# PeihaoChen/WS-MGMap

Hardware: AMD Instinct MI355X
Metric: policy steps/sec (fwd+bwd), CMA batch=8 seq=64 (higher is better)
Workload: dtype bf16

## Files before the change

include/wsmgmap.h:

```cpp
#ifndef WSMGMAP_H
#define WSMGMAP_H

#include <stdint.h>

#ifdef __cplusplus
extern "C" {
#endif

typedef void* wsmg_stream_t;

#define WSMG_EINVAL (-1)
#define WSMG_ENOMEM (-2)

int wsmg_abi_version(void);
const char* wsmg_build_info(void);


int wsmg_bev_index(const float* depth, int B, int Hd, int Wd, float depth_scale, int Hf, int Wf, int E,
                   float local_scale, int32_t* lin_idx, wsmg_stream_t stream);

int wsmg_bev_scatter_max(const float* feat, const int32_t* lin_idx, int B, int Cf, int Hf, int Wf, int C,
                         int E, float* out, wsmg_stream_t stream);

int wsmg_bev_rotate(const float* in, const float* heading, float sign, int B, int C, int E, float* out,
// ... 258 lines not shown
int wsmg_weight_relayout_bf16(const float* w_oihw, int O, int I, int KH, int KW, int I_pad, void* w_ohwi, void* w_ihwo,
                              wsmg_stream_t stream);
int wsmg_weight_grad_to_oihw(const float* dw_ohwi, int O, int I, int KH, int KW, int I_pad, float* dw_oihw,
                             wsmg_stream_t stream);

int wsmg_conv2d_bwd_weight_bf16_plan(int B, int H, int W, int Cin, int Cout, int KH, int KW, int stride, int pad, int OH, int OW,
                                     int* nsplit, long long* ws_floats);
int wsmg_conv2d_bwd_weight_bf16_slabs(const void* x, const void* dy, float* ws, int nsplit, long long ws_floats, int B, int H, int W,
                                      int Cin, int Cout, int KH, int KW, int stride, int pad, int OH, int OW, wsmg_stream_t stream);
int wsmg_conv2d_bwd_weight_plan(int B, int H, int W, int Cin, int Cout, int KH, int KW, int stride, int pad, int OH, int OW,
                                int* nsplit, long long* ws_floats);
int wsmg_conv2d_bwd_weight_slabs(const float* x, const float* dy, float* ws, int nsplit, long long ws_floats, int B, int H, int W,
                                 int Cin, int Cout, int KH, int KW, int stride, int pad, int OH, int OW, wsmg_stream_t stream);
int wsmg_weight_grad_reduce_oihw(const float* ws, int nsplit, int O, int I, int KH, int KW, int I_pad, float* dw_oihw,
                                 wsmg_stream_t stream);

int wsmg_bn_act_bwd_ld(const float* dy, int64_t ld_dy, const float* x, const float* y, const float* gamma, const float* beta,
                       const float* save_mean, const float* save_invstd, int relu, int64_t rows, int C, float* dx, float* dresidual,
                       float* dgamma, float* dbeta, double* workspace, int64_t workspace_bytes, wsmg_stream_t stream);
int wsmg_bn_act_bwd_ld_bf16(const void* dy, int64_t ld_dy, const void* x, const void* y, const float* gamma, const float* beta,
                            const float* save_mean, const float* save_invstd, int relu, int64_t rows, int C, void* dx,
                            void* dresidual, float* dgamma, float* dbeta, double* workspace, int64_t workspace_bytes,
                            wsmg_stream_t stream);
int wsmg_bn_act_bwd_ld_bf16_lo(const void* dy, int64_t ld_dy, const void* x, const void* y, const float* gamma, const float* beta,
                               const float* save_mean, const float* save_invstd, int relu, int64_t rows, int C, void* dx, void* dx_lo,
                               void* dresidual, float* dgamma, float* dbeta, double* workspace, int64_t workspace_bytes,
                               wsmg_stream_t stream);
int wsmg_relu_bwd_rows_bf16(const void* dy, int64_t ld_dy, const void* y, void* dx, int64_t rows, int C, wsmg_stream_t stream);
int wsmg_upsample2x_bwd_ld(const float* dy, int64_t ld_dy, float* dx, int B, int H, int W, int C, wsmg_stream_t stream);
int wsmg_upsample2x_bwd_ld_bf16(const void* dy, int64_t ld_dy, void* dx, int B, int H, int W, int C, wsmg_stream_t stream);
// ... 205 lines not shown
```

ws-mgmap_amd/csrc/wsmg_layout.hip:

```cpp
#include <type_traits>

#include "wsmg_common.h"

namespace {

template <bool TO_NHWC, class TI, class TO>
__global__ __launch_bounds__(256) void transpose_kernel(const TI* x, TO* y, int C_src, int HW, int C_dst) {
  __shared__ float tile[32][33];
  const int b = blockIdx.z;
  const int tx = threadIdx.x & 31, ty = threadIdx.x >> 5;
  if (TO_NHWC) {
    const int p0 = blockIdx.x * 32, c0 = blockIdx.y * 32;
#pragma unroll
    for (int j = 0; j < 4; ++j) {
      int c = c0 + ty + 8 * j, p = p0 + tx;
      tile[ty + 8 * j][tx] = (c < C_src && p < HW) ? ldf(x + ((size_t)b * C_src + c) * HW + p) : 0.f;
    }
    __syncthreads();
#pragma unroll
    for (int j = 0; j < 4; ++j) {
      int p = p0 + ty + 8 * j, c = c0 + tx;
      if (p < HW && c < C_dst) stf(y + ((size_t)b * HW + p) * C_dst + c, tile[tx][ty + 8 * j]);
    }
  } else {
// ... 75 lines not shown
  weight_relayout_body<T>(d.w_oihw, d.O, d.I, d.KH, d.KW, d.I_pad, (T*)d.w_ohwi, (T*)d.w_ihwo);
}
__global__ __launch_bounds__(256) void weight_grad_to_oihw_kernel(const float* __restrict__ dw, int O, int I, int KH, int KW,
                                                                  int I_pad, float* __restrict__ out) {
  const int64_t n = (int64_t)O * I * KH * KW;
  for (int64_t idx = (int64_t)blockIdx.x * 256 + threadIdx.x; idx < n; idx += (int64_t)gridDim.x * 256) {
    const int kw = (int)(idx % KW);
    int64_t r = idx / KW;
    const int kh = (int)(r % KH); r /= KH;
    const int i = (int)(r % I);
    const int o = (int)(r / I);
    out[idx] = dw[(((int64_t)o * KH + kh) * KW + kw) * I_pad + i];
  }
}

__global__ __launch_bounds__(256) void weight_grad_reduce_oihw_kernel(const float* __restrict__ ws, int nsplit, int64_t slab4, int I,
                                                                      int KH, int KW, int I_pad, float* __restrict__ out) {
  __shared__ f32x4 part[3][64];
  const int ql = threadIdx.x & 63, zp = threadIdx.x >> 6;
  const int64_t q = (int64_t)blockIdx.x * 64 + ql;
  const int per = (nsplit + 3) >> 2;
  const int z0 = zp * per, z1 = z0 + per < nsplit ? z0 + per : nsplit;
  f32x4 acc = {0.f, 0.f, 0.f, 0.f};
  if (q < slab4) {
    const f32x4* p = reinterpret_cast<const f32x4*>(ws) + (int64_t)z0 * slab4 + q;
    int z = z0;
    for (; z + 4 <= z1; z += 4, p += 4 * slab4) {
      const f32x4 a = p[0], b = p[slab4], c = p[2 * slab4], d = p[3 * slab4];
      acc += a; acc += b; acc += c; acc += d;
    }
    for (; z < z1; ++z, p += slab4) acc += p[0];
  }
  if (zp) part[zp - 1][ql] = acc;
  __syncthreads();
  if (zp || q >= slab4) return;
  acc += part[0][ql]; acc += part[1][ql]; acc += part[2][ql];
  const OhwiPos p = ohwi_decode(q * 4, KH, KW, I_pad);
#pragma unroll
  for (int j = 0; j < 4; ++j)
    if (p.i + j < I) out[(((int64_t)p.o * I + p.i + j) * KH + p.kh) * KW + p.kw] = acc[j];
}

template <bool TO_NHWC, class TI, class TO>
int transpose_t(const TI* x, TO* y, int B, int C_src, int H, int W, int C_dst, wsmg_stream_t stream) {
  if (B <= 0 || C_src <= 0 || C_dst <= 0 || H <= 0 || W <= 0 || B > 65535) return WSMG_EINVAL;
  int HW = H * W;
  if constexpr (TO_NHWC && std::is_same<TI, float>::value) {
    if (C_src == C_dst && C_src % 64 == 0 && HW % 4 == 0) {
      dim3 g64((unsigned)wsmg_cdiv(HW, 64), (unsigned)(C_src / 64), (unsigned)B);
      hipLaunchKernelGGL((nchw_to_nhwc64_kernel<TO>), g64, dim3(256), 0, wsmg_s(stream), x, y, C_src, HW, C_dst);
      WSMG_RETURN_LAUNCH();
    }
  }
  dim3 grid((unsigned)wsmg_cdiv(HW, 32), (unsigned)wsmg_cdiv(TO_NHWC ? C_dst : (C_dst > C_src ? C_dst : C_src), 32), (unsigned)B);
  hipLaunchKernelGGL((transpose_kernel<TO_NHWC, TI, TO>), grid, dim3(256), 0, wsmg_s(stream), x, y, C_src, HW, C_dst);
  WSMG_RETURN_LAUNCH();
}

bool weight_shape_ok(int O, int I, int KH, int KW, int I_pad) { return O > 0 && I > 0 && KH > 0 && KW > 0 && I_pad >= I; }

template <class T>
int weight_relayout_t(const float* w_oihw, int O, int I, int KH, int KW, int I_pad, T* w_ohwi, T* w_ihwo, wsmg_stream_t s) {
  if (!weight_shape_ok(O, I, KH, KW, I_pad)) return WSMG_EINVAL;
  hipLaunchKernelGGL(weight_relayout_kernel<T>, dim3(wsmg_sgrid((int64_t)O * KH * KW * I_pad)), dim3(256), 0, wsmg_s(s), w_oihw, O, I, KH,
                     KW, I_pad, w_ohwi, w_ihwo);
  WSMG_RETURN_LAUNCH();
}

}

#define B16(p) ((bf16_t*)(p))
#define CB16(p) ((const bf16_t*)(p))
extern "C" int wsmg_nchw_to_nhwc(const float* x, float* y, int B, int C_src, int H, int W, int C_dst, wsmg_stream_t s) { return transpose_t<true, float, float>(x, y, B, C_src, H, W, C_dst, s); }
extern "C" int wsmg_nchw_to_nhwc_bf16(const float* x, void* y, int B, int C_src, int H, int W, int C_dst, wsmg_stream_t s) { return transpose_t<true, float, bf16_t>(x, B16(y), B, C_src, H, W, C_dst, s); }
extern "C" int wsmg_nhwc_to_nchw(const float* x, float* y, int B, int C_src, int H, int W, int C_dst, wsmg_stream_t s) { return transpose_t<false, float, float>(x, y, B, C_src, H, W, C_dst, s); }
extern "C" int wsmg_nhwc_to_nchw_bf16(const void* x, float* y, int B, int C_src, int H, int W, int C_dst, wsmg_stream_t s) { return transpose_t<false, bf16_t, float>(CB16(x), y, B, C_src, H, W, C_dst, s); }

extern "C" int wsmg_weight_relayout(const float* w_oihw, int O, int I, int KH, int KW, int I_pad, float* w_ohwi, float* w_ihwo, wsmg_stream_t s) { return weight_relayout_t<float>(w_oihw, O, I, KH, KW, I_pad, w_ohwi, w_ihwo, s); }
extern "C" int wsmg_weight_relayout_bf16(const float* w_oihw, int O, int I, int KH, int KW, int I_pad, void* w_ohwi, void* w_ihwo, wsmg_stream_t s) { return weight_relayout_t<bf16_t>(w_oihw, O, I, KH, KW, I_pad, B16(w_ohwi), B16(w_ihwo), s); }
extern "C" int wsmg_weight_relayout_multi(const WsmgRelayoutDesc* descs, int n, int bf16, wsmg_stream_t s) {
  if (!descs || n <= 0) return WSMG_EINVAL;
// ... 5 lines not shown
      if (!weight_shape_ok(d.O, d.I, d.KH, d.KW, d.I_pad) || !d.w_oihw || !d.w_ohwi) return WSMG_EINVAL;
    }
    if (bf16) hipLaunchKernelGGL(weight_relayout_multi_kernel<bf16_t>, dim3(48, (unsigned)m), dim3(256), 0, wsmg_s(s), b);
    else hipLaunchKernelGGL(weight_relayout_multi_kernel<float>, dim3(48, (unsigned)m), dim3(256), 0, wsmg_s(s), b);
  }
  WSMG_RETURN_LAUNCH();
}
extern "C" int wsmg_weight_grad_reduce_oihw(const float* ws, int nsplit, int O, int I, int KH, int KW, int I_pad, float* dw_oihw,
                                            wsmg_stream_t s) {
  if (!ws || !dw_oihw || nsplit <= 0 || !weight_shape_ok(O, I, KH, KW, I_pad) || (I_pad & 3)) return WSMG_EINVAL;
  const int64_t slab4 = (int64_t)O * KH * KW * I_pad / 4;
  hipLaunchKernelGGL(weight_grad_reduce_oihw_kernel, dim3((unsigned)wsmg_cdiv(slab4, 64)), dim3(256), 0, wsmg_s(s), ws, nsplit, slab4, I,
                     KH, KW, I_pad, dw_oihw);
  WSMG_RETURN_LAUNCH();
}
extern "C" int wsmg_weight_grad_to_oihw(const float* dw_ohwi, int O, int I, int KH, int KW, int I_pad, float* dw_oihw, wsmg_stream_t s) {
  if (!weight_shape_ok(O, I, KH, KW, I_pad)) return WSMG_EINVAL;
  hipLaunchKernelGGL(weight_grad_to_oihw_kernel, dim3(wsmg_sgrid((int64_t)O * I * KH * KW)), dim3(256), 0, wsmg_s(s), dw_ohwi, O, I, KH, KW,
                     I_pad, dw_oihw);
  WSMG_RETURN_LAUNCH();
}
```

ws-mgmap_amd/wsmgmap/_abi.py:

```python
import ctypes
import os
import re

_HERE = os.path.dirname(os.path.abspath(__file__))
LIB_PATH = os.path.join(_HERE, "lib", "libwsmgmap.so")
if os.environ.get("WSMG_LIB"):
    LIB_PATH = os.environ["WSMG_LIB"]
HEADER_PATH = os.path.join(os.path.dirname(os.path.dirname(_HERE)), "include", "wsmgmap.h")


class WsmgError(RuntimeError):
    pass


_VALUE_TYPES = {"int": ctypes.c_int, "int32_t": ctypes.c_int, "unsigned": ctypes.c_uint, "uint32_t": ctypes.c_uint,
                "float": ctypes.c_float, "double": ctypes.c_double, "int64_t": ctypes.c_int64, "long long": ctypes.c_longlong,
                "wsmg_stream_t": ctypes.c_void_p}
_RETURN_TYPES = {"int": ctypes.c_int, "int64_t": ctypes.c_int64, "long long": ctypes.c_longlong, "const char*": ctypes.c_char_p}


def _ctype(decl, where):
    if "*" in decl:
        return ctypes.c_void_p
    ty = " ".join(decl.split()[:-1])
# ... 105 lines not shown

def take_rnn_status():
    global rnn_timeouts
    v = int(lib().wsmg_rnn_status(1))
    if v:
        rnn_timeouts += 1
    return v


def status_names(bits):
    return [n for b, n in STATUS_BITS if bits & b]


def exported_names():
    return list(_SIG)
```

ws-mgmap_amd/wsmgmap/debug.py:

```python
import os

_TABLE = [
    ("recurrent_chunks", "WSMG_RECURRENT_CHUNKS", 4, int, "time chunks of the pipelined recurrent core (wsmgmap/recurrent.py); 0 = the staged route"),
    ("rows_gemm", "WSMG_ROWS_GEMM", True, bool, "the recurrent core's dense layers as one launch each (csrc/wsmg_rows_gemm.hip); 0: the GEMM library"),
    ("fp8_fused", "WSMG_FP8_FUSED", True, bool, "ops.attention_fp8_shared as one launch (wsmg_attn_fp8_mfma_fused) where its grid barrier is safe"),
    ("fp8_row_fused", "WSMG_FP8_ROW_FUSED", True, bool, "single-query fp8 attention (one token set per row) as one launch: fold + attention per row (round 6)"),
    ("recurrent_chain", "WSMG_RECURRENT_CHAIN", True, bool, "each recurrence of the pipelined core as ONE launch chained to the attention stage by device-side counters"),
    ("decoder_streams", "WSMG_DECODER_STREAMS", 1, int, "0: map decoder on one stream; 1: side stream unless ranks share a GPU; 2: always"),
    ("early_dedup", "WSMG_EARLY_DEDUP", True, bool, "instruction dedup on its own stream when the producer marked the tokens ready (ops.mark_inputs_ready)"),
    ("early_dedup_dp", "WSMG_EARLY_DEDUP_DP", False, bool, "the early dedup also under a process group (needs the exchange on a policy stream: GradAllReducer(exchange_stream=...))"),
    ("rollout_fold", "WSMG_ROLLOUT_FOLD", True, bool, "rollout map stack with BatchNorm-folded cached operands"),
    ("depth_engine", "WSMG_DEPTH_ENGINE", False, bool, "frozen depth ResNet50 on the bf16 NHWC engine (5 % error: opt-in)"),
    ("fused_cls_tail", "WSMG_FUSED_CLS_TAIL", True, bool, "classifier tail (BN + ReLU + 1x1 + CE + pool) in one pass per direction"),
    ("bn_fused_stats", "WSMG_BN_FUSED_STATS", True, bool, "BatchNorm sums in the producing convolution's epilogue"),
    ("relu_producer_mask", "WSMG_RELU_PRODUCER_MASK", True, bool, "fused-ReLU masks of map_encoded / map_classified_linear in map_cated_linear's backward-data epilogue (round 6)"),
    ("conv_into_cat", "WSMG_CONV_INTO_CAT", True, bool, "map_encoded / map_classified_linear write straight into their slices of the concatenation (round 6)"),
    ("strided_grads", "WSMG_STRIDED_GRADS", True, bool, "channel slices of a concatenation's gradient read in place"),
    ("wgrad_atomics", "WSMG_WGRAD_ATOMICS", False, bool, "weight gradients through float atomics instead of slabs + ordered reduce (not bit-reproducible)"),
    ("conv_splitk", "WSMG_CONV_SPLITK", True, bool, "split-K for rollout-size layers"),
    ("rows_linear", "WSMG_ROWS_LINEAR", True, bool, "one-launch dense layers for <= 16 rows"),
    ("bev_fused", "WSMG_BEV_FUSED", True, bool, "scatter + rotation in one launch, plane-consuming fuse"),
    ("bev_compact", "WSMG_BEV_COMPACT", True, bool, "BEV: the index launch packs the valid sources and the scatter walks only those (round 6)"),
    ("bev_one_launch", "WSMG_BEV_ONE_LAUNCH", -1, int, "BEV: index + scatter + rotation as one launch (wsmg_bev_project) and fuse + retrieve as one (wsmg_map_fuse_retrieve); -1: where profiles/bev_fuse_retrieve.txt has them measured and not slower (fuse + retrieve at B = 1 of E = 100, C = 64, G = 240), 0: never, 1: wherever the shapes allow"),
    ("rnn_stock", "WSMG_RNN_STOCK", False, bool, "the three recurrences on the stock (MIOpen) GRU / LSTM: no persistent kernel at all (bench.py's last fallback; needs recurrent_chunks = 0)"),
    ("rnn_poison", "WSMG_RNN_POISON", False, bool, "NaN-fill the persistent kernels' workspaces first (stress tool)"),
    ("feeder_pin", "WSMG_FEEDER_PIN", True, bool, "register the feeder's shared-memory ring as pinned memory"),
    ("keep_blas", "WSMG_KEEP_BLAS", False, bool, "leave torch's BLAS backend choice alone (default: rocBLAS)"),
]


class Switches:
    def __init__(self):
        self.reload()
# ... 20 lines not shown
```

ws-mgmap_amd/wsmgmap/graph.py:

```python
import torch

from . import _abi, ops
from .common.aux_losses import AuxLosses


def _eager_dedup(owner, enc, tokens, first_call, reuse=False):
    if owner._dd_stream is None:
        owner._dd_stream = torch.cuda.Stream()
    cur = torch.cuda.current_stream()
    if first_call:
        owner._dd_stream.wait_stream(cur)
    with torch.cuda.stream(owner._dd_stream):
        dd = enc.dedup(tokens, reuse=reuse)
    cur.wait_stream(owner._dd_stream)
    for t in dd:
        if t.is_cuda:
            t.record_stream(cur)
    return dd


class GraphedAct:

    def __init__(self, policy, eager_calls=2):
        self.policy = policy
# ... 183 lines not shown
        self._bump_versions()
        rnn_hidden_states.copy_(g["h_out"])
        return g["loss"]

    def _capture(self, observations, rnn_hidden_states, prev_actions, masks, weights, dd):
        obs_s = {k: self._adopt(v) for k, v in observations.items() if torch.is_tensor(v)}
        prev_actions, masks, weights = self._adopt(prev_actions), self._adopt(masks), self._adopt(weights)
        dd_s = (dd[0].clone(), dd[1].clone(), dd[2].clone(), dd[3].clone())
        h_in = rnn_hidden_states.clone()
        obs_c = dict(obs_s)
        obs_c["instruction_dedup"] = dd_s
        torch.cuda.synchronize()
        graph = torch.cuda.CUDAGraph()
        with torch.cuda.graph(graph):
            loss, h_out = self._update(obs_c, h_in, prev_actions, masks, weights)
        if hasattr(self.optimizer, "note_replayed_steps"):
            self.optimizer.note_replayed_steps(-1)
        ops.check_rnn_status()
        return dict(graph=graph, obs=obs_s, dd=dd_s, h_in=h_in, prev=prev_actions, masks=masks, weights=weights, loss=loss, h_out=h_out)
```

ws-mgmap_amd/wsmgmap/ops/conv.py:

```python
import ctypes

import torch

from .. import _abi
from ..debug import sw
from .core import _p, _raw_stream, _stream, _req, _f32, _sfx, _workspace, _rows_of, _conv_out, _launch, _zeros_f32, _prelaid, _join_side_at_end, TokenGradSink
from .nhwc import cat_channels
from .norm import channel_sum



def prelayout_conv_weights(weights, dtype):
    descs, keep = [], []
    for w in weights:
        if w.dim() != 4 or not w.is_cuda or w.dtype != torch.float32 or not w.is_contiguous():
            continue
        O, I, KH, KW = w.shape
        cin_pad = (I + 31) // 32 * 32
        key = (w.data_ptr(), w._version, cin_pad, dtype)
        if key in _prelaid:
            continue
        ohwi = torch.empty(O, KH, KW, cin_pad, device=w.device, dtype=dtype)
        ihwo = torch.empty(cin_pad, KH, KW, O, device=w.device, dtype=dtype)
        _prelaid[key] = (ohwi, ihwo)
# ... 25 lines not shown

_wgrad_ws = {}


def _wgrad_workspace(device, floats):
    key = (device.index, _raw_stream())
    ws = _wgrad_ws.get(key)
    if ws is None or ws.numel() < floats:
        if ws is not None:
            ws.record_stream(torch.cuda.current_stream())
        ws = torch.empty(max(int(floats), 1 << 24), device=device, dtype=torch.float32)
        _wgrad_ws[key] = ws
    return ws


def _weight_grad(sfx, x, dy, dims, fl, Cin_w):
    B, H, W, Cin, Cout, KH, KW, stride, pad, OH, OW = dims
    if sw.wgrad_atomics:
        dw_ohwi = _zeros_f32((Cout, KH, KW, Cin), x.device)
        _launch("wsmg_conv2d_bwd_weight" + sfx, fl, _p(x), _p(dy), _p(dw_ohwi), *dims, _stream())
        return _weight_grad_oihw(dw_ohwi, Cin_w)
    nsplit, floats = ctypes.c_int(0), ctypes.c_longlong(0)
    _abi.call("wsmg_conv2d_bwd_weight" + sfx + "_plan", *dims, ctypes.cast(ctypes.byref(nsplit), ctypes.c_void_p),
              ctypes.cast(ctypes.byref(floats), ctypes.c_void_p))
    ws = _wgrad_workspace(x.device, floats.value)
    _launch("wsmg_conv2d_bwd_weight" + sfx + "_slabs", fl, _p(x), _p(dy), _p(ws), nsplit.value, floats.value, *dims, _stream())
    out = torch.empty(Cout, Cin_w, KH, KW, device=x.device, dtype=torch.float32)
    _launch("wsmg_weight_grad_reduce_oihw", 0.0, _p(ws), nsplit.value, Cout, Cin_w, KH, KW, Cin, _p(out), _stream(),
            prof_as="wsmg_conv2d_bwd_weight" + sfx + "_slabs")
    return out


class ReluSink:

    def __init__(self):
        self.relu = False
        self.masked = False


def _mask_of(mask_z, mask_sinks):
    if mask_z is None or not mask_sinks or not sw.relu_producer_mask or not all(m.relu for m in mask_sinks):
        return None
    for m in mask_sinks:
# ... 21 lines not shown
            _launch("wsmg_conv2d_fwd_bf16_ex", fl, _p(x), _p(w), _p(bias), ctypes.c_void_p(base.data_ptr() + c_off * 2), 2 if relu else 0,
                    None, 0, base.shape[-1], *dims, _stream())
        else:
            y = torch.empty(B, OH, OW, Cout, device=x.device, dtype=x.dtype)
            if sfx and stats is not None:
                _launch("wsmg_conv2d_fwd_bf16_stats", fl, _p(x), _p(w), _p(bias), _p(y), 2 if relu else 0, _p(stats), stats.shape[0],
                        *dims, _stream())
            elif sfx:
                _launch("wsmg_conv2d_fwd_bf16", fl, _p(x), _p(w), _p(bias), _p(y), 2 if relu else 0, *dims, _stream())
            else:
                _launch("wsmg_conv2d_fwd", fl, _p(x), _p(w), _p(bias), _p(y), *dims, _stream())
                if relu:
                    _abi.call("wsmg_relu_fwd", _p(y), _p(y), y.numel(), _stream())
        ctx.save_for_backward(x, w_ihwo, y if relu else None)
        ctx.cfg = dims + (bias is not None, sfx, Cin_w)
        ctx.bias_grad_zero = bool(bias_grad_zero)
        ctx.relu_sink = relu_sink if relu else None
        if ctx.relu_sink is not None:
            relu_sink.relu = True
        ctx.lo_sink = lo_sink if sfx else None
        return y

    @staticmethod
    def backward(ctx, dy):
        x, w_ihwo, y_relu = ctx.saved_tensors
        *dims, has_bias, sfx, Cin_w = ctx.cfg
        B, H, W, Cin, Cout, KH, KW, stride, pad, OH, OW = dims
        if ctx.relu_sink is not None and ctx.relu_sink.masked:
            y_relu = None
        if y_relu is not None:
# ... 5 lines not shown
                _abi.call("wsmg_relu_bwd_rows_bf16", _p(dy), ld, _p(y_relu), _p(masked), dy.numel() // Cout, Cout, _stream())
            else:
                _abi.call("wsmg_relu_bwd" + sfx, _p(dy), _p(y_relu), _p(masked), dy.numel(), _stream())
            dy = masked
        else:
            dy = dy.contiguous()
        dx = dw = db = None
        fl = 2.0 * B * OH * OW * Cout * Cin * KH * KW
        if ctx.needs_input_grad[0]:
            dx = torch.empty_like(x)
            if sfx:
                _launch("wsmg_conv2d_bwd_data_bf16", fl, _p(dy), _p(w_ihwo), _p(dx), 0, *dims, _stream())
            else:
                _launch("wsmg_conv2d_bwd_data", fl, _p(dy), _p(w_ihwo), _p(dx), *dims, _stream())
        if ctx.needs_input_grad[1]:
            dw = _weight_grad(sfx, x, dy, dims, fl, Cin_w)
            lo = ctx.lo_sink.take() if ctx.lo_sink is not None else None
            if lo is not None and lo.shape == dy.shape:
                dw = dw + _weight_grad(sfx, x, lo, dims, fl, Cin_w)
        if has_bias and ctx.needs_input_grad[2]:
            db = _zeros_f32((Cout,), dy.device) if ctx.bias_grad_zero else channel_sum(dy.view(-1, Cout))
        return dx, dw, db, None, None, None, None, None, None, None, None


class _ConvT2d(torch.autograd.Function):

    @staticmethod
    def forward(ctx, x, w_iohw, stride, pad, stats=None):
        _req(x, w_iohw)
        _f32(w_iohw)
        sfx = _sfx(x)
        B, Hs, Ws, Ct_in = x.shape
        O, I, KH, KW = w_iohw.shape
        assert O == Ct_in
        Hb, Wb = (Hs - 1) * stride - 2 * pad + KH, (Ws - 1) * stride - 2 * pad + KW
        w, w_ihwo = _weight_layouts(w_iohw.contiguous(), I, x.dtype, True)
        y = torch.empty(B, Hb, Wb, I, device=x.device, dtype=x.dtype)
        fl = 2.0 * B * Hs * Ws * O * I * KH * KW
        dims = (B, Hb, Wb, I, O, KH, KW, stride, pad, Hs, Ws)
        if sfx and stats is not None:
            _launch("wsmg_conv2d_bwd_data_bf16_stats", fl, _p(x), _p(w_ihwo), _p(y), 0, _p(stats), stats.shape[0], *dims, _stream())
        elif sfx:
            _launch("wsmg_conv2d_bwd_data_bf16", fl, _p(x), _p(w_ihwo), _p(y), 0, *dims, _stream())
        else:
            _launch("wsmg_conv2d_bwd_data", fl, _p(x), _p(w_ihwo), _p(y), *dims, _stream())
        ctx.save_for_backward(x, w)
        ctx.cfg = dims + (sfx,)
        return y

    @staticmethod
    def backward(ctx, dy):
        x, w = ctx.saved_tensors
        *dims, sfx = ctx.cfg
        B, Hb, Wb, I, O, KH, KW, stride, pad, Hs, Ws = dims
        dy = dy.contiguous()
        dx = dw = None
        fl = 2.0 * B * Hs * Ws * O * I * KH * KW
        if ctx.needs_input_grad[0]:
            dx = torch.empty_like(x)
            if sfx:
                _launch("wsmg_conv2d_fwd_bf16", fl, _p(dy), _p(w), None, _p(dx), 0, *dims, _stream())
            else:
                _launch("wsmg_conv2d_fwd", fl, _p(dy), _p(w), None, _p(dx), *dims, _stream())
        if ctx.needs_input_grad[1]:
            dw = _weight_grad(sfx, dy, x, tuple(dims), fl, I)
        return dx, dw, None, None, None


def conv2d(x, weight_oihw, bias, stride=1, pad=0, bias_grad_zero=False, relu=False, stats=None, relu_sink=None, into=None, lo_sink=None):
    return _Conv2d.apply(x, weight_oihw, bias, stride, pad, bias_grad_zero, relu, stats, relu_sink, into, lo_sink)


class _Conv2dCat2(torch.autograd.Function):

    @staticmethod
    def forward(ctx, a, b, base, w_oihw, bias, relu, relu_sink, mask_sinks):
        _req(base, w_oihw, bias)
        _f32(w_oihw, bias)
        B, H, W, Cin = base.shape
        Cout, Cin_w, KH, KW = w_oihw.shape
        assert Cin == Cin_w and KH == 3 and KW == 3 and base.dtype == torch.bfloat16
        w, w_ihwo = _weight_layouts(w_oihw.contiguous(), Cin, base.dtype, True)
        y = torch.empty(B, H, W, Cout, device=base.device, dtype=base.dtype)
        fl = 2.0 * B * H * W * Cout * Cin * 9
        dims = (B, H, W, Cin, Cout, 3, 3, 1, 1, H, W)
        _launch("wsmg_conv2d_fwd_bf16", fl, _p(base), _p(w), _p(bias), _p(y), 2 if relu else 0, *dims, _stream())
        ctx.save_for_backward(base, w_ihwo, y if relu else None)
        ctx.cfg = dims + (bias is not None, a.shape[-1])
        ctx.relu_sink = relu_sink if relu else None
        if ctx.relu_sink is not None:
            relu_sink.relu = True
        ctx.mask_sinks = mask_sinks
        return y

    @staticmethod
    def backward(ctx, dy):
        base, w_ihwo, y_relu = ctx.saved_tensors
        *dims, has_bias, ca = ctx.cfg
        B, H, W, Cin, Cout = dims[:5]
        if ctx.relu_sink is not None and ctx.relu_sink.masked:
            y_relu = None
        if y_relu is not None:
            masked = torch.empty_like(y_relu)
            dy = dy.contiguous()
            _abi.call("wsmg_relu_bwd_bf16", _p(dy), _p(y_relu), _p(masked), dy.numel(), _stream())
            dy = masked
        else:
            dy = dy.contiguous()
        fl = 2.0 * B * H * W * Cout * Cin * 9
        da = torch.empty(B, H, W, ca, device=dy.device, dtype=dy.dtype)
        db = torch.empty(B, H, W, Cin - ca, device=dy.device, dtype=dy.dtype)
        _launch("wsmg_conv2d_bwd_data_bf16_ex", fl, _p(dy), _p(w_ihwo), _p(da), _p(_mask_of(base, ctx.mask_sinks)), _p(db), ca, *dims, _stream())
        dw = _weight_grad("_bf16", base, dy, tuple(dims), fl, Cin) if ctx.needs_input_grad[3] else None
        dbias = channel_sum(dy.view(-1, Cout)) if (has_bias and ctx.needs_input_grad[4]) else None
        return da, db, None, dw, dbias, None, None, None


def conv2d_over_written_parts(a, b, base, weight_oihw, bias, relu=True, relu_sink=None, mask_sinks=None):
    ca, cb = a.shape[-1], b.shape[-1]
    ok = (base.dtype == torch.bfloat16 and base.is_contiguous() and base.shape[-1] == ca + cb and ca % 8 == 0 and cb % 8 == 0
          and a.data_ptr() == base.data_ptr() and b.data_ptr() == base.data_ptr() + ca * base.element_size()
          and a.stride() == base.stride() and b.stride() == base.stride() and tuple(weight_oihw.shape[1:]) == (ca + cb, 3, 3))
    if not ok:
        return conv2d(cat_channels(a.contiguous(), b.contiguous()), weight_oihw, bias, 1, 1, relu=relu, relu_sink=relu_sink)
    return _Conv2dCat2.apply(a, b, base, weight_oihw, bias, relu, relu_sink, mask_sinks)


def conv2d_cat(xs, weight_oihw, bias, stride=1, pad=0, bias_grad_zero=False, relu=False, relu_sink=None):
# ... 81 lines not shown
```

ws-mgmap_amd/wsmgmap/ops/core.py:

```python
import ctypes

import torch

from .. import _abi
from ..debug import sw

_ws_cache = {}


def _p(t):
    return None if t is None else ctypes.c_void_p(t.data_ptr())


if hasattr(torch._C, "_cuda_getCurrentRawStream") and hasattr(torch._C, "_cuda_getDevice"):
    def _raw_stream():
        return torch._C._cuda_getCurrentRawStream(torch._C._cuda_getDevice())
else:
    def _raw_stream():
        return torch.cuda.current_stream().cuda_stream


def _stream():
    return ctypes.c_void_p(_raw_stream())

# ... 198 lines not shown
_prelaid = {}


_zero_pool = {}


def _zero_pool_retire():
    for z in _zero_pool.values():
        z["cap"] = max(z["cap"], z["used"])
        z["buf"], z["off"], z["used"], z["armed"] = None, 0, 0, False


chain_in_flight = False


def reset_pass_state():
    global chain_in_flight
    chain_in_flight = False
    TokenGradSink.check_none_pending()
    _prelaid.clear()
    if any(z["armed"] for z in _zero_pool.values()):
        _zero_pool_retire()
    if _side_join_armed:
        for main_id, side_id in list(_side_join_armed):
            for side in _leaf_streams:
                if side.cuda_stream == side_id:
                    torch.cuda.current_stream().wait_stream(side)
        _side_join_armed.clear()


def _zeros_f32(shape, device):
    numel = 1
    for d in shape:
        numel *= int(d)
    n = (numel + 63) // 64 * 64
# ... 68 lines not shown
```

ws-mgmap_amd/wsmgmap/optim.py:

```python
import collections
import ctypes
import inspect
import math

import torch

from . import _abi


_AdamDesc = _abi.AdamDesc

ADAM_CHUNK = 4096
ADAM_MAX = 48
FLAG_AMSGRAD, FLAG_MAXIMIZE, FLAG_DECOUPLED_WD = 1, 2, 4
_TORCH_HAS_DECOUPLED = "decoupled_weight_decay" in inspect.signature(torch.optim.Adam.__init__).parameters
HYPER_ROW = 8


def _check_max_grad_norm(max_grad_norm):
    if max_grad_norm is not None and not (math.isfinite(max_grad_norm) and max_grad_norm > 0.0):
        raise ValueError(f"invalid max_grad_norm: {max_grad_norm} (a finite positive number, or None for no clipping)")


def _check_hyper(lr, betas, eps, weight_decay):
# ... 56 lines not shown


def _checked_grad_descs(what, grads):
    some = [g for g in grads if g is not None]
    if not some:
        raise _abi.WsmgError(f"wsmgmap.optim.{what}: no parameter has a gradient")
    dev = some[0].device
    for g in some:
        if g.is_sparse or not (g.is_cuda and g.dtype == torch.float32 and g.device == dev):
            raise _abi.WsmgError(f"wsmgmap.optim.{what}: gradients must be dense float32 CUDA tensors on one device")
    grads = [g if g is None or g.is_contiguous() else g.contiguous() for g in grads]
    return dev, _grad_descs(grads), grads


def grad_stats(params):
    dev, descs, grads = _checked_grad_descs("grad_stats", [p.grad for p in params])
    with torch.cuda.device(dev):
        cap = max(1, _norm_blocks(descs))
        partials = torch.empty(cap, device=dev, dtype=torch.float64)
        scan = torch.empty(4 * cap, device=dev, dtype=torch.int32)
        report = torch.empty(len(grads), 4, device=dev, dtype=torch.int32)
        _abi.call("wsmg_grad_stats_multi", descs, len(grads), _ptr(partials), cap, _ptr(scan), cap, _ptr(report), _stream(dev))
    return report


def global_grad_norm(params):
    dev, descs, grads = _checked_grad_descs("global_grad_norm", [p.grad for p in params if p.grad is not None])
    with torch.cuda.device(dev):
        guard = torch.zeros(4, device=dev, dtype=torch.float32)
        cap = max(1, _norm_blocks(descs))
        partials = torch.empty(cap, device=dev, dtype=torch.float64)
        _abi.call("wsmg_grad_norm_multi", descs, len(grads), _ptr(partials), cap, 0.0, 0, _ptr(guard), None, _stream(dev))
    return guard[0]


class Adam(torch.optim.Optimizer):
    def __init__(self, params, lr=1e-3, betas=(0.9, 0.999), eps=1e-8, weight_decay=0.0, amsgrad=False, maximize=False,
                 capturable=False, max_grad_norm=None, skip_nonfinite=False, guard_buffers=None, hyper_on_device=False,
                 grad_report=False, decoupled_weight_decay=False):
        self._capturable = bool(capturable)
        self._step_dev = {}
# ... 288 lines not shown
        b1, b2 = group["betas"]
        by_value = (float(group["lr"]), float(b1), float(b2), float(group["eps"]), float(group["weight_decay"]))
        if guard is not None:
            _abi.call("wsmg_adam_step_multi_guarded" + ext, descs, n, *more, *by_value, sd, guard, stream)
        elif sd is not None:
            _abi.call("wsmg_adam_step_multi_dev" + ext, descs, n, *more, *by_value, sd, stream)
        else:
            _abi.call("wsmg_adam_step_multi" + ext, descs, n, *more, *by_value, 1.0 - b1 ** step, 1.0 - b2 ** step, stream)

    @torch.no_grad()
    def step(self, closure=None):
        loss = None
        if closure is not None:
            with torch.enable_grad():
                loss = closure()
        if self._hyper_on_device:
            self._hyper_before_step()
        if self._guarded:
            self._guarded_step()
            return loss
        for gi, group in enumerate(self.param_groups):
            by_step = {}
            for item, step in zip(*self._stepped_items(group)[:2]):
                by_step.setdefault(step, []).append(item)
            if self._capturable and len(by_step) > 1:
                raise _abi.WsmgError("wsmgmap.optim.Adam(capturable=True): the stepped parameters of a group must share one step count")
            for step, items in by_step.items():
                dev = items[0][0].device
                with torch.cuda.device(dev):
                    if self._hyper_on_device and self._hyper.device != dev:
# ... 146 lines not shown
```

ws-mgmap_amd/wsmgmap/parallel.py:

```python
import time
import zlib

import torch
import torch.distributed as dist


class GradExchangeError(RuntimeError):
    pass


class GradAllReducer:
    def __init__(self, params, bucket_bytes=8 << 20, group=None, single_rank_exchange=False, module=None, broadcast_buffers_every=0,
                 exchange_stream=None):
        self._xstream = exchange_stream
        self._restore = []
        if exchange_stream is not None:
            from . import debug
            self._restore.append((debug.sw, "early_dedup_dp", debug.sw.early_dedup_dp))
            debug.sw.early_dedup_dp = True
        self._module = module
        self._buffers_every = int(broadcast_buffers_every)
        if self._buffers_every > 0 and module is None:
            raise ValueError("broadcast_buffers_every needs the module whose buffers are to be broadcast")
        self._updates = 0
# ... 144 lines not shown

    def _note(self, msg):
        if self._local_error is None:
            self._local_error = msg

    def _exchange_stream(self):
        xs = self._xstream
        if isinstance(xs, str):
            from . import ops
            xs = self._xstream = ops.helper_stream(xs, device=self.params[0].device)
        return xs

    def _launch(self, bi):
        b = self._buckets[bi]
        xs = self._exchange_stream() if b["params"][0].is_cuda else None
        if b["params"][0].is_cuda:
            cur = xs if xs is not None else torch.cuda.current_stream()
            for sid, st in b.pop("streams", {}).items():
                if sid != cur.cuda_stream:
                    ev = torch.cuda.Event()
                    ev.record(st)
                    cur.wait_event(ev)
        grads = []
        for q, v in zip(b["params"], b["views"]):
            if q.grad is None:
                grads.append(torch.zeros_like(v))
            elif q.grad.data_ptr() == v.data_ptr():
                grads.append(None)
            else:
                grads.append(q.grad)
# ... 202 lines not shown
```

Before: 50610.

## Defer bf16 weight-gradient slab reductions into one grouped launch per backward

```diff
diff --git a/include/wsmgmap.h b/include/wsmgmap.h
--- a/include/wsmgmap.h
+++ b/include/wsmgmap.h
@@ -296,6 +296,13 @@
                                  int Cin, int Cout, int KH, int KW, int stride, int pad, int OH, int OW, wsmg_stream_t stream);
 int wsmg_weight_grad_reduce_oihw(const float* ws, int nsplit, int O, int I, int KH, int KW, int I_pad, float* dw_oihw,
                                  wsmg_stream_t stream);
+#define WSMG_WGRAD_FINISH_MAX 32
+int wsmg_wgrad_finish_multi(const float* const* slabs, float* const* dst, const long long* slab_stride, const int* dims, int n,
+                            wsmg_stream_t stream);
+int wsmg_wgrad_finish_plan(const float* const* slabs, float* const* dst, const long long* slab_stride, const int* dims, int n,
+                           int* launches, int* first_unit);
+int wsmg_wgrad_finish_entry_of(const int* first_unit, int n, int unit);
+int wsmg_wgrad_arena_take(long long cap_floats, long long* used_floats, long long want_floats, long long* offset_floats);
 
 int wsmg_bn_act_bwd_ld(const float* dy, int64_t ld_dy, const float* x, const float* y, const float* gamma, const float* beta,
                        const float* save_mean, const float* save_invstd, int relu, int64_t rows, int C, float* dx, float* dresidual,
diff --git a/ws-mgmap_amd/csrc/wsmg_layout.hip b/ws-mgmap_amd/csrc/wsmg_layout.hip
--- a/ws-mgmap_amd/csrc/wsmg_layout.hip
+++ b/ws-mgmap_amd/csrc/wsmg_layout.hip
@@ -1,4 +1,5 @@
 #include <type_traits>
+#include <vector>
 
 #include "wsmg_common.h"
 
@@ -113,22 +114,22 @@
   }
 }
 
-__global__ __launch_bounds__(256) void weight_grad_reduce_oihw_kernel(const float* __restrict__ ws, int nsplit, int64_t slab4, int I,
-                                                                      int KH, int KW, int I_pad, float* __restrict__ out) {
-  __shared__ f32x4 part[3][64];
+__device__ __forceinline__ void weight_grad_reduce_unit(const float* __restrict__ ws, int nsplit, int64_t stride4, int64_t slab4,
+                                                        int64_t unit, int I, int KH, int KW, int I_pad, float* __restrict__ out,
+                                                        f32x4 (*part)[64]) {
   const int ql = threadIdx.x & 63, zp = threadIdx.x >> 6;
-  const int64_t q = (int64_t)blockIdx.x * 64 + ql;
+  const int64_t q = unit * 64 + ql;
   const int per = (nsplit + 3) >> 2;
   const int z0 = zp * per, z1 = z0 + per < nsplit ? z0 + per : nsplit;
   f32x4 acc = {0.f, 0.f, 0.f, 0.f};
   if (q < slab4) {
-    const f32x4* p = reinterpret_cast<const f32x4*>(ws) + (int64_t)z0 * slab4 + q;
+    const f32x4* p = reinterpret_cast<const f32x4*>(ws) + (int64_t)z0 * stride4 + q;
     int z = z0;
-    for (; z + 4 <= z1; z += 4, p += 4 * slab4) {
-      const f32x4 a = p[0], b = p[slab4], c = p[2 * slab4], d = p[3 * slab4];
+    for (; z + 4 <= z1; z += 4, p += 4 * stride4) {
+      const f32x4 a = p[0], b = p[stride4], c = p[2 * stride4], d = p[3 * stride4];
       acc += a; acc += b; acc += c; acc += d;
     }
-    for (; z < z1; ++z, p += slab4) acc += p[0];
+    for (; z < z1; ++z, p += stride4) acc += p[0];
   }
   if (zp) part[zp - 1][ql] = acc;
   __syncthreads();
@@ -138,6 +139,38 @@
 #pragma unroll
   for (int j = 0; j < 4; ++j)
     if (p.i + j < I) out[(((int64_t)p.o * I + p.i + j) * KH + p.kh) * KW + p.kw] = acc[j];
+}
+__global__ __launch_bounds__(256) void weight_grad_reduce_oihw_kernel(const float* __restrict__ ws, int nsplit, int64_t slab4, int I,
+                                                                      int KH, int KW, int I_pad, float* __restrict__ out) {
+  __shared__ f32x4 part[3][64];
+  weight_grad_reduce_unit(ws, nsplit, slab4, slab4, blockIdx.x, I, KH, KW, I_pad, out, part);
+}
+struct WsmgWgradFinishDesc {
+  const float* slabs;
+  float* dst;
+  long long slab_stride;
+  int n_split, Cout, Cin, KH, KW, Cin_pad;
+};
+struct WgradFinishBatch {
+  WsmgWgradFinishDesc d[WSMG_WGRAD_FINISH_MAX];
+  int first_unit[WSMG_WGRAD_FINISH_MAX + 1];
+  int n;
+};
+__host__ __device__ inline int wgrad_finish_entry_of(const int* first_unit, int n, int unit) {
+  int lo = 0, hi = n - 1;
+  while (lo < hi) {
+    const int mid = (lo + hi + 1) >> 1;
+    if (first_unit[mid] <= unit) lo = mid; else hi = mid - 1;
+  }
+  return lo;
+}
+__global__ __launch_bounds__(256) void weight_grad_reduce_oihw_multi_kernel(WgradFinishBatch b) {
+  __shared__ f32x4 part[3][64];
+  const int t = wgrad_finish_entry_of(b.first_unit, b.n, (int)blockIdx.x);
+  const WsmgWgradFinishDesc& d = b.d[t];
+  const int64_t slab4 = (int64_t)d.Cout * d.KH * d.KW * d.Cin_pad / 4;
+  weight_grad_reduce_unit(d.slabs, d.n_split, d.slab_stride / 4, slab4, (int)blockIdx.x - b.first_unit[t], d.Cin, d.KH, d.KW, d.Cin_pad,
+                          d.dst, part);
 }
 
 template <bool TO_NHWC, class TI, class TO>
@@ -164,6 +197,35 @@
   hipLaunchKernelGGL(weight_relayout_kernel<T>, dim3(wsmg_sgrid((int64_t)O * KH * KW * I_pad)), dim3(256), 0, wsmg_s(s), w_oihw, O, I, KH,
                      KW, I_pad, w_ohwi, w_ihwo);
   WSMG_RETURN_LAUNCH();
+}
+
+bool wgrad_finish_desc_ok(const WsmgWgradFinishDesc& d) {
+  if (!d.slabs || !d.dst || d.n_split <= 0 || !weight_shape_ok(d.Cout, d.Cin, d.KH, d.KW, d.Cin_pad) || (d.Cin_pad & 3)) return false;
+  return d.slab_stride >= (long long)d.Cout * d.KH * d.KW * d.Cin_pad && !(d.slab_stride & 3) && !((uintptr_t)d.slabs & 15);
+}
+bool wgrad_finish_gather(const float* const* slabs, float* const* dst, const long long* slab_stride, const int* dims, int n,
+                         std::vector<WsmgWgradFinishDesc>& out) {
+  if (!slabs || !dst || !slab_stride || !dims || n < 0) return false;
+  out.resize((size_t)n);
+  for (int i = 0; i < n; ++i) {
+    const int* d = dims + 6 * i;
+    out[i] = WsmgWgradFinishDesc{slabs[i], dst[i], slab_stride[i], d[0], d[1], d[2], d[3], d[4], d[5]};
+    if (!wgrad_finish_desc_ok(out[i])) return false;
+  }
+  return true;
+}
+int64_t wgrad_finish_units(const WsmgWgradFinishDesc& d) { return wsmg_cdiv((int64_t)d.Cout * d.KH * d.KW * d.Cin_pad / 4, 64); }
+int64_t wgrad_finish_fill(const WsmgWgradFinishDesc* descs, int m, WgradFinishBatch& b) {
+  int64_t units = 0;
+  b.n = m;
+  for (int i = 0; i < m; ++i) {
+    b.d[i] = descs[i];
+    b.first_unit[i] = (int)units;
+    units += wgrad_finish_units(descs[i]);
+    if (units > 0x7fffffff) return -1;
+  }
+  for (int i = m; i <= WSMG_WGRAD_FINISH_MAX; ++i) b.first_unit[i] = (int)units;
+  return units;
 }
 
 }
@@ -199,6 +261,47 @@
                      KH, KW, I_pad, dw_oihw);
   WSMG_RETURN_LAUNCH();
 }
+extern "C" int wsmg_wgrad_finish_multi(const float* const* slabs, float* const* dst, const long long* slab_stride, const int* dims, int n,
+                                       wsmg_stream_t s) {
+  if (n == 0) return 0;
+  std::vector<WsmgWgradFinishDesc> descs;
+  if (!wgrad_finish_gather(slabs, dst, slab_stride, dims, n, descs)) return WSMG_EINVAL;
+  for (int i0 = 0; i0 < n; i0 += WSMG_WGRAD_FINISH_MAX) {
+    WgradFinishBatch b{};
+    if (wgrad_finish_fill(descs.data() + i0, n - i0 < WSMG_WGRAD_FINISH_MAX ? n - i0 : WSMG_WGRAD_FINISH_MAX, b) < 0) return WSMG_EINVAL;
+  }
+  for (int i0 = 0; i0 < n; i0 += WSMG_WGRAD_FINISH_MAX) {
+    WgradFinishBatch b{};
+    const int64_t units = wgrad_finish_fill(descs.data() + i0, n - i0 < WSMG_WGRAD_FINISH_MAX ? n - i0 : WSMG_WGRAD_FINISH_MAX, b);
+    hipLaunchKernelGGL(weight_grad_reduce_oihw_multi_kernel, dim3((unsigned)units), dim3(256), 0, wsmg_s(s), b);
+  }
+  WSMG_RETURN_LAUNCH();
+}
+extern "C" int wsmg_wgrad_finish_plan(const float* const* slabs, float* const* dst, const long long* slab_stride, const int* dims, int n,
+                                      int* launches, int* first_unit) {
+  if (!launches || n < 0 || (n && !first_unit)) return WSMG_EINVAL;
+  *launches = 0;
+  std::vector<WsmgWgradFinishDesc> descs;
+  if (n && !wgrad_finish_gather(slabs, dst, slab_stride, dims, n, descs)) return WSMG_EINVAL;
+  for (int i0 = 0; i0 < n; i0 += WSMG_WGRAD_FINISH_MAX, ++*launches) {
+    WgradFinishBatch b{};
+    if (wgrad_finish_fill(descs.data() + i0, n - i0 < WSMG_WGRAD_FINISH_MAX ? n - i0 : WSMG_WGRAD_FINISH_MAX, b) < 0) return WSMG_EINVAL;
+    for (int i = 0; i <= WSMG_WGRAD_FINISH_MAX; ++i) first_unit[*launches * (WSMG_WGRAD_FINISH_MAX + 1) + i] = b.first_unit[i];
+  }
+  return 0;
+}
+extern "C" int wsmg_wgrad_finish_entry_of(const int* first_unit, int n, int unit) {
+  if (!first_unit || n <= 0 || n > WSMG_WGRAD_FINISH_MAX || unit < 0 || unit >= first_unit[n]) return WSMG_EINVAL;
+  return wgrad_finish_entry_of(first_unit, n, unit);
+}
+extern "C" int wsmg_wgrad_arena_take(long long cap_floats, long long* used_floats, long long want_floats, long long* offset_floats) {
+  if (!used_floats || !offset_floats || cap_floats < 0 || want_floats <= 0 || *used_floats < 0 || (*used_floats & 63)) return WSMG_EINVAL;
+  const long long want = (want_floats + 63) / 64 * 64;
+  if (*used_floats + want > cap_floats) return WSMG_ENOMEM;
+  *offset_floats = *used_floats;
+  *used_floats += want;
+  return 0;
+}
 extern "C" int wsmg_weight_grad_to_oihw(const float* dw_ohwi, int O, int I, int KH, int KW, int I_pad, float* dw_oihw, wsmg_stream_t s) {
   if (!weight_shape_ok(O, I, KH, KW, I_pad)) return WSMG_EINVAL;
   hipLaunchKernelGGL(weight_grad_to_oihw_kernel, dim3(wsmg_sgrid((int64_t)O * I * KH * KW)), dim3(256), 0, wsmg_s(s), dw_ohwi, O, I, KH, KW,
diff --git a/ws-mgmap_amd/wsmgmap/_abi.py b/ws-mgmap_amd/wsmgmap/_abi.py
--- a/ws-mgmap_amd/wsmgmap/_abi.py
+++ b/ws-mgmap_amd/wsmgmap/_abi.py
@@ -143,3 +143,14 @@
 
 def exported_names():
     return list(_SIG)
+
+
+def wgrad_finish_args(entries):
+    n = len(entries)
+    slabs, dst = (ctypes.c_void_p * max(n, 1))(), (ctypes.c_void_p * max(n, 1))()
+    stride, dims = (ctypes.c_longlong * max(n, 1))(), (ctypes.c_int * (6 * max(n, 1)))()
+    for i, e in enumerate(entries):
+        slabs[i], dst[i], stride[i] = e[0], e[1], e[2]
+        dims[6 * i:6 * i + 6] = e[3:9]
+    arrays = (slabs, dst, stride, dims)
+    return tuple(ctypes.cast(a, ctypes.c_void_p) for a in arrays) + (n,), arrays
diff --git a/ws-mgmap_amd/wsmgmap/debug.py b/ws-mgmap_amd/wsmgmap/debug.py
--- a/ws-mgmap_amd/wsmgmap/debug.py
+++ b/ws-mgmap_amd/wsmgmap/debug.py
@@ -17,6 +17,7 @@
     ("conv_into_cat", "WSMG_CONV_INTO_CAT", True, bool, "map_encoded / map_classified_linear write straight into their slices of the concatenation (round 6)"),
     ("strided_grads", "WSMG_STRIDED_GRADS", True, bool, "channel slices of a concatenation's gradient read in place"),
     ("wgrad_atomics", "WSMG_WGRAD_ATOMICS", False, bool, "weight gradients through float atomics instead of slabs + ordered reduce (not bit-reproducible)"),
+    ("wgrad_finish", "WSMG_WGRAD_FINISH", "grouped", str, "bf16 weight gradients' ordered slab sums: 'grouped' = one launch at the end of the backward pass (ops.flush_weight_grads; a hook on another tensor that reads a conv parameter's .grad inside the pass must call it first), 'layer' = one launch per layer"),
     ("conv_splitk", "WSMG_CONV_SPLITK", True, bool, "split-K for rollout-size layers"),
     ("rows_linear", "WSMG_ROWS_LINEAR", True, bool, "one-launch dense layers for <= 16 rows"),
     ("bev_fused", "WSMG_BEV_FUSED", True, bool, "scatter + rotation in one launch, plane-consuming fuse"),
diff --git a/ws-mgmap_amd/wsmgmap/graph.py b/ws-mgmap_amd/wsmgmap/graph.py
--- a/ws-mgmap_amd/wsmgmap/graph.py
+++ b/ws-mgmap_amd/wsmgmap/graph.py
@@ -221,6 +221,7 @@
         graph = torch.cuda.CUDAGraph()
         with torch.cuda.graph(graph):
             loss, h_out = self._update(obs_c, h_in, prev_actions, masks, weights)
+            ops.flush_weight_grads()
         if hasattr(self.optimizer, "note_replayed_steps"):
             self.optimizer.note_replayed_steps(-1)
         ops.check_rnn_status()
diff --git a/ws-mgmap_amd/wsmgmap/ops/conv.py b/ws-mgmap_amd/wsmgmap/ops/conv.py
--- a/ws-mgmap_amd/wsmgmap/ops/conv.py
+++ b/ws-mgmap_amd/wsmgmap/ops/conv.py
@@ -4,7 +4,7 @@
 
 from .. import _abi
 from ..debug import sw
-from .core import _p, _raw_stream, _stream, _req, _f32, _sfx, _workspace, _rows_of, _conv_out, _launch, _zeros_f32, _prelaid, _join_side_at_end, TokenGradSink
+from .core import _p, _raw_stream, _stream, _req, _f32, _sfx, _workspace, _rows_of, _conv_out, _launch, _zeros_f32, _prelaid, _join_side_at_end, TokenGradSink, _pass_reset_hooks
 from .nhwc import cat_channels
 from .norm import channel_sum
 
@@ -63,7 +63,89 @@
     return ws
 
 
-def _weight_grad(sfx, x, dy, dims, fl, Cin_w):
+_wgrad_arenas = {}
+_wgrad_pending = []
+_wgrad_pending_params = set()
+_wgrad_flush_armed = False
+wgrad_finish_stats = {"grouped": 0, "layer": 0, "flushes": 0}
+
+
+def _wgrad_arena_take(device, floats):
+    key = (device.index, _raw_stream())
+    a = _wgrad_arenas.get(key)
+    if a is None:
+        guess = max([o["learned"] for k, o in _wgrad_arenas.items() if k[0] == device.index], default=0)
+        a = _wgrad_arenas[key] = dict(buf=None, used=ctypes.c_longlong(0), want=0, learned=guess)
+    need = (floats + 63) // 64 * 64
+    a["want"] += need
+    cap = 0 if a["buf"] is None else a["buf"].numel()
+    if a["used"].value == 0 and cap < max(a["learned"], need) and a["learned"]:
+        a["buf"] = torch.empty(max(a["learned"], need), device=device, dtype=torch.float32)
+        cap = a["buf"].numel()
+    off = ctypes.c_longlong(0)
+    rc = _abi.lib().wsmg_wgrad_arena_take(cap, ctypes.cast(ctypes.byref(a["used"]), ctypes.c_void_p), floats,
+                                          ctypes.cast(ctypes.byref(off), ctypes.c_void_p))
+    if rc == -2:
+        return None, a
+    if rc != 0:
+        raise _abi.WsmgError(f"wsmg_wgrad_arena_take failed: {rc}")
+    return ctypes.c_void_p(a["buf"].data_ptr() + 4 * off.value), a
+
+
+def flush_weight_grads():
+    if not _wgrad_pending:
+        return
+    pending = list(_wgrad_pending)
+    _wgrad_pending.clear()
+    _wgrad_pending_params.clear()
+    by_dev = {}
+    for desc, keep, stream in pending:
+        by_dev.setdefault(stream.device, []).append((desc, stream))
+    for dev, items in by_dev.items():
+        with torch.cuda.device(dev):
+            cur = torch.cuda.current_stream()
+            for sid, st in {s.cuda_stream: s for _, s in items}.items():
+                if sid != cur.cuda_stream:
+                    cur.wait_stream(st)
+            args, arrays = _abi.wgrad_finish_args([d for d, _ in items])
+            _abi.call("wsmg_wgrad_finish_multi", *args, _stream())
+            wgrad_finish_stats["flushes"] += 1
+
+
+def _wgrad_end_of_pass():
+    global _wgrad_flush_armed
+    _wgrad_flush_armed = False
+    flush_weight_grads()
+    for a in _wgrad_arenas.values():
+        a["learned"], a["want"] = max(a["learned"], a["want"]), 0
+        a["used"].value = 0
+
+
+def _wgrad_reset_pass():
+    if _wgrad_flush_armed:
+        _wgrad_end_of_pass()
+
+
+_pass_reset_hooks.append(_wgrad_reset_pass)
+
+
+def _wgrad_defer(param):
+    global _wgrad_flush_armed
+    if (sw.wgrad_finish != "grouped" or param is None or not param.is_leaf or param.grad is not None or id(param) in _wgrad_pending_params
+            or param._backward_hooks or getattr(param, "_post_accumulate_grad_hooks", None)):
+        return False
+    if torch.distributed.is_available() and torch.distributed.is_initialized() and torch.distributed.get_world_size() > 1:
+        return False
+    if not _wgrad_flush_armed:
+        try:
+            torch.autograd.Variable._execution_engine.queue_callback(_wgrad_end_of_pass)
+        except RuntimeError:
+            return False
+        _wgrad_flush_armed = True
+    return True
+
+
+def _weight_grad(sfx, x, dy, dims, fl, Cin_w, param=None):
     B, H, W, Cin, Cout, KH, KW, stride, pad, OH, OW = dims
     if sw.wgrad_atomics:
         dw_ohwi = _zeros_f32((Cout, KH, KW, Cin), x.device)
@@ -72,10 +154,21 @@
     nsplit, floats = ctypes.c_int(0), ctypes.c_longlong(0)
     _abi.call("wsmg_conv2d_bwd_weight" + sfx + "_plan", *dims, ctypes.cast(ctypes.byref(nsplit), ctypes.c_void_p),
               ctypes.cast(ctypes.byref(floats), ctypes.c_void_p))
-    ws = _wgrad_workspace(x.device, floats.value)
-    _launch("wsmg_conv2d_bwd_weight" + sfx + "_slabs", fl, _p(x), _p(dy), _p(ws), nsplit.value, floats.value, *dims, _stream())
+    ws = arena = None
+    if sfx and _wgrad_defer(param):
+        ws, arena = _wgrad_arena_take(x.device, floats.value)
+    deferred = ws is not None
+    if not deferred:
+        ws = _p(_wgrad_workspace(x.device, floats.value))
+    wgrad_finish_stats["grouped" if deferred else "layer"] += 1
+    _launch("wsmg_conv2d_bwd_weight" + sfx + "_slabs", fl, _p(x), _p(dy), ws, nsplit.value, floats.value, *dims, _stream())
     out = torch.empty(Cout, Cin_w, KH, KW, device=x.device, dtype=torch.float32)
-    _launch("wsmg_weight_grad_reduce_oihw", 0.0, _p(ws), nsplit.value, Cout, Cin_w, KH, KW, Cin, _p(out), _stream(),
+    if deferred:
+        desc = (ws.value, out.data_ptr(), floats.value // nsplit.value, nsplit.value, Cout, Cin_w, KH, KW, Cin)
+        _wgrad_pending.append((desc, (out.untyped_storage(), arena["buf"]), torch.cuda.current_stream()))
+        _wgrad_pending_params.add(id(param))
+        return out
+    _launch("wsmg_weight_grad_reduce_oihw", 0.0, ws, nsplit.value, Cout, Cin_w, KH, KW, Cin, _p(out), _stream(),
             prof_as="wsmg_conv2d_bwd_weight" + sfx + "_slabs")
     return out
 
@@ -127,6 +220,7 @@
                     _abi.call("wsmg_relu_fwd", _p(y), _p(y), y.numel(), _stream())
         ctx.save_for_backward(x, w_ihwo, y if relu else None)
         ctx.cfg = dims + (bias is not None, sfx, Cin_w)
+        ctx.w_param = w_oihw
         ctx.bias_grad_zero = bool(bias_grad_zero)
         ctx.relu_sink = relu_sink if relu else None
         if ctx.relu_sink is not None:
@@ -162,8 +256,8 @@
             else:
                 _launch("wsmg_conv2d_bwd_data", fl, _p(dy), _p(w_ihwo), _p(dx), *dims, _stream())
         if ctx.needs_input_grad[1]:
-            dw = _weight_grad(sfx, x, dy, dims, fl, Cin_w)
             lo = ctx.lo_sink.take() if ctx.lo_sink is not None else None
+            dw = _weight_grad(sfx, x, dy, dims, fl, Cin_w, None if lo is not None else ctx.w_param)
             if lo is not None and lo.shape == dy.shape:
                 dw = dw + _weight_grad(sfx, x, lo, dims, fl, Cin_w)
         if has_bias and ctx.needs_input_grad[2]:
@@ -194,6 +288,7 @@
             _launch("wsmg_conv2d_bwd_data", fl, _p(x), _p(w_ihwo), _p(y), *dims, _stream())
         ctx.save_for_backward(x, w)
         ctx.cfg = dims + (sfx,)
+        ctx.w_param = w_iohw
         return y
 
     @staticmethod
@@ -211,7 +306,7 @@
             else:
                 _launch("wsmg_conv2d_fwd", fl, _p(dy), _p(w), None, _p(dx), *dims, _stream())
         if ctx.needs_input_grad[1]:
-            dw = _weight_grad(sfx, dy, x, tuple(dims), fl, I)
+            dw = _weight_grad(sfx, dy, x, tuple(dims), fl, I, ctx.w_param)
         return dx, dw, None, None, None
 
 
@@ -235,6 +330,7 @@
         _launch("wsmg_conv2d_fwd_bf16", fl, _p(base), _p(w), _p(bias), _p(y), 2 if relu else 0, *dims, _stream())
         ctx.save_for_backward(base, w_ihwo, y if relu else None)
         ctx.cfg = dims + (bias is not None, a.shape[-1])
+        ctx.w_param = w_oihw
         ctx.relu_sink = relu_sink if relu else None
         if ctx.relu_sink is not None:
             relu_sink.relu = True
@@ -259,7 +355,7 @@
         da = torch.empty(B, H, W, ca, device=dy.device, dtype=dy.dtype)
         db = torch.empty(B, H, W, Cin - ca, device=dy.device, dtype=dy.dtype)
         _launch("wsmg_conv2d_bwd_data_bf16_ex", fl, _p(dy), _p(w_ihwo), _p(da), _p(_mask_of(base, ctx.mask_sinks)), _p(db), ca, *dims, _stream())
-        dw = _weight_grad("_bf16", base, dy, tuple(dims), fl, Cin) if ctx.needs_input_grad[3] else None
+        dw = _weight_grad("_bf16", base, dy, tuple(dims), fl, Cin, ctx.w_param) if ctx.needs_input_grad[3] else None
         dbias = channel_sum(dy.view(-1, Cout)) if (has_bias and ctx.needs_input_grad[4]) else None
         return da, db, None, dw, dbias, None, None, None
 
diff --git a/ws-mgmap_amd/wsmgmap/ops/core.py b/ws-mgmap_amd/wsmgmap/ops/core.py
--- a/ws-mgmap_amd/wsmgmap/ops/core.py
+++ b/ws-mgmap_amd/wsmgmap/ops/core.py
@@ -236,11 +236,16 @@
 chain_in_flight = False
 
 
+_pass_reset_hooks = []
+
+
 def reset_pass_state():
     global chain_in_flight
     chain_in_flight = False
     TokenGradSink.check_none_pending()
     _prelaid.clear()
+    for hook in _pass_reset_hooks:
+        hook()
     if any(z["armed"] for z in _zero_pool.values()):
         _zero_pool_retire()
     if _side_join_armed:
diff --git a/ws-mgmap_amd/wsmgmap/optim.py b/ws-mgmap_amd/wsmgmap/optim.py
--- a/ws-mgmap_amd/wsmgmap/optim.py
+++ b/ws-mgmap_amd/wsmgmap/optim.py
@@ -6,6 +6,7 @@
 import torch
 
 from . import _abi
+from .ops.conv import flush_weight_grads
 
 
 _AdamDesc = _abi.AdamDesc
@@ -94,6 +95,7 @@
 
 
 def grad_stats(params):
+    flush_weight_grads()
     dev, descs, grads = _checked_grad_descs("grad_stats", [p.grad for p in params])
     with torch.cuda.device(dev):
         cap = max(1, _norm_blocks(descs))
@@ -105,6 +107,7 @@
 
 
 def global_grad_norm(params):
+    flush_weight_grads()
     dev, descs, grads = _checked_grad_descs("global_grad_norm", [p.grad for p in params if p.grad is not None])
     with torch.cuda.device(dev):
         guard = torch.zeros(4, device=dev, dtype=torch.float32)
@@ -423,6 +426,7 @@
         if closure is not None:
             with torch.enable_grad():
                 loss = closure()
+        flush_weight_grads()
         if self._hyper_on_device:
             self._hyper_before_step()
         if self._guarded:
diff --git a/ws-mgmap_amd/wsmgmap/parallel.py b/ws-mgmap_amd/wsmgmap/parallel.py
--- a/ws-mgmap_amd/wsmgmap/parallel.py
+++ b/ws-mgmap_amd/wsmgmap/parallel.py
@@ -182,6 +182,9 @@
     def _launch(self, bi):
         b = self._buckets[bi]
         xs = self._exchange_stream() if b["params"][0].is_cuda else None
+        if b["params"][0].is_cuda:
+            from .ops.conv import flush_weight_grads
+            flush_weight_grads()
         if b["params"][0].is_cuda:
             cur = xs if xs is not None else torch.cuda.current_stream()
             for sid, st in b.pop("streams", {}).items():
```

New measurement: 50760, median of 6. Within noise of the previous version (+0.3%).
